# megvii-research/basedet

Hardware: AMD Instinct MI355X
Metric: images/sec training RetinaNet-R50-FPN 1333x800 (higher is better)
Workload: dtype bf16; 1 GPU; retinanet_r50_800x1344 train step (fwd+bwd+allreduce+SGD), DummyLoader boxes, random-init weights, inputs resident in HBM; per_gpu_batch=16, global_batch=16, parallelism=dp1

## Files before the change

basedet_amd/csrc/gskip.hip:

```cpp
#include "common.h"

namespace {

enum { GS_ANY = 1, GS_TOP = 2, GS_BOT = 4, GS_LEFT = 8, GS_RIGHT = 16, GS_TL = 32, GS_TR = 64, GS_BL = 128, GS_BR = 256 };

struct GsSeg { int patch_start, H, W, pw, off; };

struct GsParams {
    const bf16_raw* g;
    int* mask;
    int C, ppi, ph, pw_px, nseg, patches_per_img, total;
    GsSeg seg[BD_MAX_SEGS];
};

__device__ __forceinline__ int gs_level(const GsParams& p, int rem) {
    int s = 0;
#pragma unroll
    for (int k = 1; k < BD_MAX_SEGS; ++k)
        if (k < p.nseg && rem >= p.seg[k].patch_start) s = k;
    return s;
}

__global__ __launch_bounds__(256) void gskip_scan_kernel(const GsParams p) {
    __shared__ int sbits;
    const int tid = threadIdx.x;
    const int pid = blockIdx.x;
    const int n = pid / p.patches_per_img, rem = pid - n * p.patches_per_img;
    const int s = gs_level(p, rem);
    const int H = p.seg[s].H, W = p.seg[s].W, pwn = p.seg[s].pw;
    const int local = rem - p.seg[s].patch_start, by = local / pwn, bx = local - by * pwn;
    const int y0 = by * p.ph, x0 = bx * p.pw_px;
    const int cpp = p.C >> 3;
    const int items = p.ph * p.pw_px * cpp;
    const long long img = (long long)n * p.ppi + p.seg[s].off;
    if (tid == 0) sbits = 0;
    __syncthreads();
    int bits = 0;
    constexpr int U = 8;
    for (int b = 0; b < items; b += 256 * U) {
        u32x4_t v[U];
        int pix[U];
#pragma unroll
        for (int k = 0; k < U; ++k) {
            const int i = b + k * 256 + tid;
            v[k] = (u32x4_t){0u, 0u, 0u, 0u};
            pix[k] = -1;
            if (i < items) {
                const int px = i / cpp, ch = i - px * cpp;
                const int py = px / p.pw_px, pxx = px - py * p.pw_px;
                const int y = y0 + py, x = x0 + pxx;
                if (y < H && x < W) {
                    v[k] = *reinterpret_cast<const u32x4_t*>(p.g + (img + (long long)y * W + x) * p.C + ch * 8);
                    pix[k] = px;
                }
            }
        }
#pragma unroll
        for (int k = 0; k < U; ++k) {
            if (pix[k] >= 0 && (v[k][0] | v[k][1] | v[k][2] | v[k][3])) {
                const int py = pix[k] / p.pw_px, pxx = pix[k] - py * p.pw_px;
                const bool t = py == 0, bo = py == p.ph - 1, l = pxx == 0, r = pxx == p.pw_px - 1;
                bits |= GS_ANY | (t ? GS_TOP : 0) | (bo ? GS_BOT : 0) | (l ? GS_LEFT : 0) | (r ? GS_RIGHT : 0) | (t && l ? GS_TL : 0) |
                        (t && r ? GS_TR : 0) | (bo && l ? GS_BL : 0) | (bo && r ? GS_BR : 0);
            }
        }
    }
#pragma unroll
    for (int m = 32; m >= 1; m >>= 1) bits |= __shfl_xor(bits, m, 64);
    if ((tid & 63) == 0 && bits) atomicOr(&sbits, bits);
    __syncthreads();
    if (tid == 0) p.mask[pid] = sbits;
}

template <bool FRESH>
__device__ __forceinline__ int gs_mask(const int* m, int i) {
    if (FRESH) return __hip_atomic_load(m + i, __ATOMIC_RELAXED, __HIP_MEMORY_SCOPE_AGENT);
    return m[i];
}

template <bool FRESH>
__device__ __forceinline__ void gs_compact_body(const GsParams& p, int* live, int* list, int* count, int* wsum) {
    constexpr int KP = 8;
    const int tid = threadIdx.x, wv = tid >> 6, ln = tid & 63;
    int base = 0;
    for (int c0 = 0; c0 < p.total; c0 += 1024 * KP) {
        int lv[KP];
#pragma unroll
        for (int j = 0; j < KP; ++j) {
            const int q = c0 + tid * KP + j;
            lv[j] = 0;
            if (q < p.total) {
                const int n = q / p.patches_per_img, rem = q - n * p.patches_per_img;
                const int s = gs_level(p, rem);
                const int pwn = p.seg[s].pw, rows = (p.seg[s].H + p.ph - 1) / p.ph;
                const int local = rem - p.seg[s].patch_start, by = local / pwn, bx = local - by * pwn;
                const int* m = p.mask + (long long)n * p.patches_per_img + p.seg[s].patch_start;
                const bool up = by > 0, dn = by + 1 < rows, lf = bx > 0, rt = bx + 1 < pwn;
                int v = gs_mask<FRESH>(m, by * pwn + bx) & GS_ANY;
                if (up) v |= gs_mask<FRESH>(m, (by - 1) * pwn + bx) & GS_BOT;
                if (dn) v |= gs_mask<FRESH>(m, (by + 1) * pwn + bx) & GS_TOP;
                if (lf) v |= gs_mask<FRESH>(m, by * pwn + bx - 1) & GS_RIGHT;
                if (rt) v |= gs_mask<FRESH>(m, by * pwn + bx + 1) & GS_LEFT;
                if (up && lf) v |= gs_mask<FRESH>(m, (by - 1) * pwn + bx - 1) & GS_BR;
                if (up && rt) v |= gs_mask<FRESH>(m, (by - 1) * pwn + bx + 1) & GS_BL;
                if (dn && lf) v |= gs_mask<FRESH>(m, (by + 1) * pwn + bx - 1) & GS_TR;
                if (dn && rt) v |= gs_mask<FRESH>(m, (by + 1) * pwn + bx + 1) & GS_TL;
                lv[j] = v != 0;
            }
        }
        int cnt = 0;
#pragma unroll
        for (int j = 0; j < KP; ++j) cnt += lv[j];
        int inc = cnt;
#pragma unroll
        for (int o = 1; o < 64; o <<= 1) {
            const int y = __shfl_up(inc, o, 64);
            if (ln >= o) inc += y;
        }
        if (ln == 63) wsum[wv] = inc;
        __syncthreads();
        int off = base + inc - cnt, tot = 0;
#pragma unroll
        for (int w = 0; w < 16; ++w) {
            off += w < wv ? wsum[w] : 0;
            tot += wsum[w];
        }
#pragma unroll
        for (int j = 0; j < KP; ++j) {
            const int q = c0 + tid * KP + j;
            if (q < p.total) live[q] = lv[j];
            if (lv[j]) list[off++] = q;
        }
        base += tot;
        __syncthreads();
    }
    if (tid == 0) *count = base;
}

__global__ __launch_bounds__(1024) void gskip_compact_kernel(const GsParams p, int* live, int* list, int* count) {
    __shared__ int wsum[16];
    gs_compact_body<false>(p, live, list, count, wsum);
}

enum { GM_HDR = 8 };

struct GmSeg { int H, W, off, s4, s8, ss; };

struct GmParams {
    const bf16_raw* t;
    const int* live_in;
    int* map;
    int C, ppi, nseg, pi4, pi8, pis, tot4, tot8;
    GmSeg seg[BD_MAX_SEGS];
};

__global__ __launch_bounds__(1024) void gskip_fill_kernel(const GmParams p, const GsParams cp, int total) {
    __shared__ int sbits, slast;
    __shared__ int wsum[16];
    const int tid = threadIdx.x;
    int* m4 = p.map + GM_HDR;
    int* m8 = m4 + p.tot4;
    const int cpp = p.C >> 3;
    const int items = 4 * 16 * cpp;
    for (int pid = blockIdx.x; pid < total; pid += gridDim.x) {
        const int n = pid / p.pis, rem = pid - n * p.pis;
        int s = 0;
#pragma unroll
        for (int k = 1; k < BD_MAX_SEGS; ++k)
            if (k < p.nseg && rem >= p.seg[k].ss) s = k;
        const int H = p.seg[s].H, W = p.seg[s].W;
        const int sc = (W + 15) >> 4, r4 = (H + 3) >> 2, c8 = (W + 7) >> 3;
        const int local = rem - p.seg[s].ss, sy = local / sc, sx = local - sy * sc;
        int q4[2], q8[2];
        bool ok4[2], ok8[2], lv[2];
#pragma unroll
        for (int h = 0; h < 2; ++h) {
            ok4[h] = 2 * sy + h < r4;
            q4[h] = n * p.pi4 + p.seg[s].s4 + (2 * sy + h) * sc + sx;
            ok8[h] = 2 * sx + h < c8;
            q8[h] = n * p.pi8 + p.seg[s].s8 + sy * c8 + 2 * sx + h;
            lv[h] = ok4[h] && (p.live_in == nullptr || p.live_in[q4[h]] != 0);
        }
        int b = 0;
        if (lv[0] || lv[1]) {
            if (tid == 0) sbits = 0;
            __syncthreads();
            const long long img = (long long)n * p.ppi + p.seg[s].off;
            int bits = 0;
#pragma unroll
            for (int h = 0; h < 2; ++h) {
                if (!lv[h]) continue;
                for (int i = tid; i < items; i += 1024) {
                    const int px = i / cpp, ch = i - px * cpp;
                    const int py = px >> 4, pxx = px & 15;
                    const int y = 8 * sy + 4 * h + py, x = 16 * sx + pxx;
                    if (y < H && x < W) {
                        const u32x4_t v = *reinterpret_cast<const u32x4_t*>(p.t + (img + (long long)y * W + x) * p.C + ch * 8);
                        if (v[0] | v[1] | v[2] | v[3]) {
                            const bool t = py == 0, bo = py == 3, l = pxx == 0, r = pxx == 15;
                            const int w = GS_ANY | (t ? GS_TOP : 0) | (bo ? GS_BOT : 0) | (l ? GS_LEFT : 0) | (r ? GS_RIGHT : 0) |
                                          (t && l ? GS_TL : 0) | (t && r ? GS_TR : 0) | (bo && l ? GS_BL : 0) | (bo && r ? GS_BR : 0);
                            bits |= (w << (9 * h)) | (1 << (18 + (pxx >> 3)));
                        }
                    }
                }
            }
#pragma unroll
            for (int m = 32; m >= 1; m >>= 1) bits |= __shfl_xor(bits, m, 64);
            if ((tid & 63) == 0 && bits) atomicOr(&sbits, bits);
            __syncthreads();
            b = sbits;
            __syncthreads();
        }
        if (tid == 0) {
            if (ok4[0]) m4[q4[0]] = b & 511;
            if (ok4[1]) m4[q4[1]] = (b >> 9) & 511;
            if (ok8[0]) m8[q8[0]] = (b >> 18) & 1;
            if (ok8[1]) m8[q8[1]] = (b >> 19) & 1;
        }
    }
    if (tid == 0) {
        __builtin_amdgcn_fence(__ATOMIC_RELEASE, "agent");
        slast = atomicAdd(p.map + 1, 1) == (int)gridDim.x - 1;
    }
    __syncthreads();
    if (!slast) return;
    __builtin_amdgcn_fence(__ATOMIC_ACQUIRE, "agent");
    const int nxt = (p.map[0] & 1) ^ 1;
    int* live = m8 + p.tot8;
    gs_compact_body<true>(cp, live, live + p.tot4 * (1 + nxt), p.map + 2 + nxt, wsum);
    if (tid == 0) { p.map[0] = nxt; p.map[1] = 0; }
}

GsParams gs_params(const bd_conv_desc* d, int ph, int pw, int side = 0) {
    GsParams p{};
    p.C = side ? d->Cin : d->Cout; p.ppi = side ? d->in_pix_per_img : d->out_pix_per_img; p.ph = ph; p.pw_px = pw; p.nseg = d->nseg;
    int ps = 0;
    for (int s = 0; s < d->nseg; ++s) {
        GsSeg& sg = p.seg[s];
        const int H = side ? d->Hi[s] : d->Ho[s], W = side ? d->Wi[s] : d->Wo[s];
        sg.patch_start = ps; sg.H = H; sg.W = W; sg.pw = cdiv(W, pw); sg.off = side ? d->in_off[s] : d->out_off[s];
        ps += cdiv(H, ph) * sg.pw;
    }
    p.patches_per_img = ps;
    p.total = ps * d->N;
    return p;
}

}

int bd_gskip_patches(const bd_conv_desc* d, int ph, int pw) {
    return gs_params(d, ph, pw).total;
}

void bd_gskip_scan(const bd_conv_desc* d, const void* g, int ph, int pw, int* mask, hipStream_t stream) {
    GsParams p = gs_params(d, ph, pw);
    p.g = (const bf16_raw*)g; p.mask = mask;
    if (p.total > 0) hipLaunchKernelGGL(gskip_scan_kernel, dim3(p.total), dim3(256), 0, stream, p);
}

void bd_gskip_compact(const bd_conv_desc* d, int ph, int pw, const int* mask, int* live, int* list, int* count, hipStream_t stream) {
    GsParams p = gs_params(d, ph, pw);
    p.mask = const_cast<int*>(mask);
    hipLaunchKernelGGL(gskip_compact_kernel, dim3(1), dim3(1024), 0, stream, p, live, list, count);
}

void bd_gskip_map_layout(const bd_conv_desc* d, int side, BdGskipMap* out) {
    const int p4 = gs_params(d, 4, 16, side).total, p8 = gs_params(d, 8, 8, side).total;
    out->p4 = p4; out->p8 = p8;
    out->m4 = GM_HDR; out->m8 = GM_HDR + p4; out->live = out->m8 + p8; out->list = out->live + p4;
    out->ints = (size_t)GM_HDR + (size_t)4 * p4 + p8;
}

extern "C" size_t bd_conv2d_gskip_map_bytes(const bd_conv_desc* d, int of_dx) {
    if (!d || d->nseg < 1 || d->nseg > BD_MAX_SEGS || !(d->R == 3 && d->S == 3 && d->stride == 1 && d->pad == 1)) return 0;
    BdGskipMap m;
    bd_gskip_map_layout(d, of_dx ? 1 : 0, &m);
    return m.ints * sizeof(int);
}

void bd_gskip_fill(const bd_conv_desc* d, int side, const void* t, const int* live_in, int* map, hipStream_t stream) {
    const GsParams g4 = gs_params(d, 4, 16, side), g8 = gs_params(d, 8, 8, side), gs = gs_params(d, 8, 16, side);
    GmParams p{};
    p.t = (const bf16_raw*)t; p.live_in = live_in; p.map = map;
    p.C = g4.C; p.ppi = g4.ppi; p.nseg = g4.nseg;
    p.pi4 = g4.patches_per_img; p.pi8 = g8.patches_per_img; p.pis = gs.patches_per_img; p.tot4 = g4.total; p.tot8 = g8.total;
    for (int s = 0; s < g4.nseg; ++s)
        p.seg[s] = GmSeg{g4.seg[s].H, g4.seg[s].W, g4.seg[s].off, g4.seg[s].patch_start, g8.seg[s].patch_start, gs.seg[s].patch_start};
    GsParams cp = g4;
    cp.mask = map + GM_HDR;
    const int grid = gs.total < 128 ? gs.total : 128;
    if (grid > 0) hipLaunchKernelGGL(gskip_fill_kernel, dim3(grid), dim3(1024), 0, stream, p, cp, gs.total);
}

extern "C" int bd_gskip_map_scan(const bd_conv_desc* d, int of_dx, const void* t, void* map, size_t map_bytes, bd_stream_t stream) {
    BD_REQUIRE(d && t && map, "gskip_map_scan: null pointer");
    const size_t need = bd_conv2d_gskip_map_bytes(d, of_dx);
    BD_REQUIRE(need > 0, "gskip_map_scan: liveness maps belong to 3x3 / stride 1 / pad 1 descriptors");
    BD_REQUIRE(map_bytes >= need, "gskip_map_scan: map %zu < required %zu bytes", map_bytes, need);
    const int side = of_dx ? 1 : 0;
    BdGskipMap m;
    bd_gskip_map_layout(d, side, &m);
    int* mp = (int*)map;
    if (hipMemsetAsync(mp, 0, GM_HDR * sizeof(int), (hipStream_t)stream) != hipSuccess) { bd_set_error("gskip_map_scan: memset failed"); return BD_ELAUNCH; }
    GsParams p4 = gs_params(d, 4, 16, side), p8 = gs_params(d, 8, 8, side);
    p4.g = p8.g = (const bf16_raw*)t;
    p4.mask = mp + m.m4; p8.mask = mp + m.m8;
    if (p4.total > 0) {
        hipLaunchKernelGGL(gskip_scan_kernel, dim3(p4.total), dim3(256), 0, (hipStream_t)stream, p4);
        hipLaunchKernelGGL(gskip_scan_kernel, dim3(p8.total), dim3(256), 0, (hipStream_t)stream, p8);
    }
    hipLaunchKernelGGL(gskip_compact_kernel, dim3(1), dim3(1024), 0, (hipStream_t)stream, p4, mp + m.live, mp + m.list, mp + 2);
    BD_CHECK_LAUNCH("bd_gskip_map_scan");
    return BD_OK;
}
```

basedet_amd/layers/modules.py:

```python
import torch

from .. import ops


def _to_nchw(t, N, H, W, C=None):
    v = t.float().view(N, H, W, -1).permute(0, 3, 1, 2).contiguous()
    return v if C is None else v[:, :C].contiguous()


def _level(t, geom, i, C=None):
    N = geom.N
    v = t.view(N, geom.pix_per_img, -1)[:, geom.off[i]: geom.off[i] + geom.H[i] * geom.W[i]]
    return _to_nchw(v.contiguous(), N, geom.H[i], geom.W[i], C)


class _Trunk:
    def __init__(self, cfg, params=None, model=None):
        if model is None:
            from ..models import FCOS, FasterRCNN, RetinaNet
            kind = {"FCOS": FCOS, "ATSS": FCOS, "OTA": FCOS, "FasterRCNN": FasterRCNN}.get(cfg.MODEL.NAME, RetinaNet)
            model = kind(cfg, params=params)
        self.model = model
        self.cfg = cfg

    def _run_trunk(self, image):
        m = self.model
        pre = m.pre_process({"data": image})
        pl = pre["plan"]
        head_forward, m.head_forward = m.head_forward, (lambda _pl: None)
        try:
            m.network_forward(pl)
        finally:
            m.head_forward = head_forward
        return pl


class FPN(_Trunk):

    def __call__(self, image):
        pl = self._run_trunk(image)
        names = self.cfg.MODEL.FPN.OUT_FEATURES
        return {n: _level(pl.P, pl.pyr, i) for i, n in enumerate(names)}

    def output_shape(self):
        ch = self.cfg.MODEL.FPN.OUT_CHANNELS
        return {n: dict(channels=ch, stride=s) for n, s in zip(self.cfg.MODEL.FPN.OUT_FEATURES, self.cfg.MODEL.FPN.STRIDES)}


def build_backbone(cfg, params=None):
    return FPN(cfg, params=params)


class _ResNet(_Trunk):

    def __call__(self, image):
        pl = self._run_trunk(image)
        m = self.model
        out = {}
        for i, blk in enumerate(m.blocks):
            last = i + 1 == len(m.blocks) or m.blocks[i + 1]["layer"] != blk["layer"]
            if last:
                b = pl.blk[i]
                out[f"res{blk['layer'] + 1}"] = _to_nchw(b.out, pl.N, b.gout.H[0], b.gout.W[0])
        return out

    extract_features = __call__


def _resnet(name):
    def make(cfg=None, params=None, **kw):
        from ..configs import RetinaNetConfig
        cfg = cfg or RetinaNetConfig()
        cfg.MODEL.BACKBONE.NAME = name
        if name in ("resnet18", "resnet34"):
            cfg.MODEL.BACKBONE.OUT_FEATURE_CHANNELS = [128, 256, 512]
            cfg.MODEL.FPN.TOP_BLOCK_IN_CHANNELS = 512
        return _ResNet(cfg, params=params)
    make.__name__ = name
    make.__doc__ = f"models/cls/resnet.py: {name} feature extractor (FrozenBN, stem + res2..res5)."
    return make


resnet18, resnet34, resnet50, resnet101 = (_resnet(n) for n in ("resnet18", "resnet34", "resnet50", "resnet101"))


class _Head(_Trunk):
    def _load(self, features):
        m = self.model
        N, _, h0, w0 = features[0].shape
        s0 = m.strides[0]
        pl = m._plan(N, h0 * s0, w0 * s0)
        m._bind_plan(pl)
        assert len(features) == pl.pyr.nlev, "input features expected {}, got {}".format(pl.pyr.nlev, len(features))
        P = pl.P.view(N, pl.pyr.pix_per_img, -1)
        for i, f in enumerate(features):
            assert tuple(f.shape[2:]) == (pl.pyr.H[i], pl.pyr.W[i]), "feature sizes must follow one padded image size"
            P[:, pl.pyr.off[i]: pl.pyr.off[i] + f.shape[2] * f.shape[3]] = \
                f.permute(0, 2, 3, 1).reshape(N, -1, f.shape[1]).to(torch.bfloat16)
        return pl


def _store(dst, geom, grads, C):
    N = geom.N
    v = dst.view(N, geom.pix_per_img, -1)
    v.zero_()
    for i, g in enumerate(grads):
        assert tuple(g.shape[2:]) == (geom.H[i], geom.W[i]) and g.shape[1] == C, "gradient shapes must match the forward outputs"
        v[:, geom.off[i]: geom.off[i] + g.shape[2] * g.shape[3], :C] = g.permute(0, 2, 3, 1).reshape(N, -1, C).to(dst.dtype)


def _real_classes(conv, t):
    if conv.cls_ld == conv.K:
        return t
    return conv.real_logits(t.permute(0, 2, 3, 1)).permute(0, 3, 1, 2).contiguous()


def _pad_classes(conv, g):
    if conv.cls_ld == conv.K:
        return g
    N, _, H, W = g.shape
    out = g.new_zeros((N, conv.A, conv.cls_ld, H, W))
    out[:, :, : conv.K] = g.reshape(N, conv.A, conv.K, H, W)
    return out.reshape(N, conv.A * conv.cls_ld, H, W)


class _HeadBackward:
    def _finish(self, pl):
        m = self.model
        m._join_wgrads()
        torch.cuda.current_stream().synchronize()
        return [_level(pl.g_P, pl.pyr, i) for i in range(pl.pyr.nlev)]

    def grads(self):
        return {k: v for k, v in self.model.reference_grads().items() if k.startswith("head.")}


class RetinaNetHead(_Head, _HeadBackward):

    def __init__(self, cfg, input_shape=None, params=None, model=None):
        super().__init__(cfg, params=params, model=model)

    def __call__(self, features):
        pl = self._load(features)
        m = self.model
        m.head_forward(pl)
        n = pl.pyr.nlev
        self._pl = pl
        return ([_real_classes(m.cls_score, _level(pl.logits, pl.pyr, i)) for i in range(n)],
                [_level(pl.offsets, pl.pyr, i, m.num_anchors * 4) for i in range(n)])

    def backward(self, d_logits, d_offsets):
        pl, m = self._pl, self.model
        m._cur = pl
        m._begin_wgrads()
        assert all(g.shape[1] == m.num_anchors * m.num_classes for g in d_logits), "gradient shapes must match the forward outputs"
        _store(pl.d_logits, pl.pyr, [_pad_classes(m.cls_score, g) for g in d_logits], m.num_anchors * m.cls_ld)
        _store(pl.d_offsets, pl.pyr, d_offsets, m.num_anchors * 4)
        m.head_backward(pl, pl.wgrad_ws, pl.colsum_ws)
        return self._finish(pl)


class PointHead(_Head, _HeadBackward):

    def __init__(self, cfg, input_shape=None, params=None, model=None):
        if model is None:
            from ..models import FCOS
            model = FCOS(cfg, params=params)
        super().__init__(cfg, model=model)

    def __call__(self, features):
        pl = self._load(features)
        self.model.head_forward(pl)
        n = pl.pyr.nlev
        logits = [_level(pl.logits, pl.pyr, i, self.model.num_classes) for i in range(n)]
        offsets = [_level(pl.offsets, pl.pyr, i, 4) for i in range(n)]
        ctr = [_level(pl.raw, pl.pyr, i)[:, 4:5].contiguous() for i in range(n)]
        self._pl = pl
        return logits, offsets, ctr

    def backward(self, d_logits, d_offsets, d_ctrness):
        pl, m = self._pl, self.model
        m._cur = pl
        m._begin_wgrads()
        _store(pl.d_logits, pl.pyr, d_logits, m.num_classes)
        _store(pl.d_off, pl.pyr, d_offsets, 4)
        N = pl.pyr.N
        dc = pl.d_ctr.view(N, pl.pyr.pix_per_img)
        for i, g in enumerate(d_ctrness):
            dc[:, pl.pyr.off[i]: pl.pyr.off[i] + g.shape[2] * g.shape[3]] = g.reshape(N, -1).to(dc.dtype)
        m.head_backward(pl, pl.wgrad_ws, pl.colsum_ws)
        return self._finish(pl)
```

basedet_amd/models/retinanet.py:

```python
import torch

from .. import ops
from ..streams import fork, join
from ..utils.registry import registers
from . import params as P
from .engine import PaddedClsConv
from .fpn_base import FPNDetector, _round_up


@registers.models.register()
class RetinaNet(FPNDetector):
    @staticmethod
    def init_params(cfg, seed=0):
        return P.init_retinanet_params(cfg, seed)

    @classmethod
    def check_config(cls, cfg):
        super().check_config(cfg)
        if not cfg.MODEL.HEAD.get("WITH_NORM", True):
            raise ValueError("MODEL.HEAD.WITH_NORM = False is not supported for the RetinaNet family: only True (the default) is implemented")

    def _build_head(self, add, params):
        m = self.cfg.MODEL
        ch = self.fpn_ch
        self.num_anchors = len(m.ANCHOR.SCALES[0]) * len(m.ANCHOR.RATIOS[0])
        nc = m.HEAD.NUM_CONVS
        self.cls_tower = [add(f"head.cls_subnet.{2 * i}", ch, ch, 3, 1, 1, bias=True) for i in range(nc)]
        self.box_tower = [add(f"head.bbox_subnet.{2 * i}", ch, ch, 3, 1, 1, bias=True) for i in range(nc)]
        A, K = self.num_anchors, self.num_classes
        self.cls_score = self.convs["head.cls_score"] = PaddedClsConv("head.cls_score", ch, A, K, 3, 1, 1, self.device)
        self.cls_ld = self.cls_score.cls_ld
        self.box_ld = _round_up(A * 4, 8)
        self.bbox_pred = add("head.bbox_pred", ch, A * 4, 3, 1, 1, bias=True, cout_pad=self.box_ld)
        if bool(m.get("SPARSE_BOX_BWD", True)) and m.get("WEIGHT_DTYPE", "bf16") == "bf16":
            for c in self.box_tower + [self.bbox_pred]:
                c.gskip = True
        self.sparse_chain = bool(m.get("SPARSE_BOX_CHAIN", True))
        self._build_base_anchors()

    def _head_convs(self):
        return self.cls_tower + self.box_tower + [self.cls_score, self.bbox_pred]

    def _plan_head(self, pl):
        ch = self.fpn_ch
        N = pl.N
        C = pl._carve
        bf = torch.bfloat16

        def act(g, c):
            return C.empty((g.pixels, c), bf)

        nc = len(self.cls_tower)
        pl.cls_act = [act(pl.pyr, ch) for _ in range(nc)]
        pl.box_act = [act(pl.pyr, ch) for _ in range(nc)]
        A, K = self.num_anchors, self.num_classes
        pl.logits = act(pl.pyr, A * self.cls_ld)
        pl.offsets = act(pl.pyr, self.box_ld)
        pl.d_logits = C.like(pl.logits)
        pl.d_offsets = C.like(pl.offsets)
        pl.g_tower = [[act(pl.pyr, ch) for _ in range(nc)] for _ in range(2)]
        pl.g_map = None
        if self.sparse_chain and all(c.gskip for c in self.box_tower + [self.bbox_pred]):
            nb = ops.conv2d_gskip_map_bytes(self.box_tower[0].desc(pl.pyr, pl.pyr))
            if nb:
                pl.g_map = [C.empty(((nb + 3) // 4,), torch.int32) for _ in range(nc)]
        pl.chain_epoch = None
        tw = lambda: C.empty((pl.pyr.pixels, ch), torch.uint8)
        pl.cls_act8 = [tw() if c.fp8 else None for c in self.cls_tower]
        pl.box_act8 = [tw() if c.fp8 else None for c in self.box_tower]
        tg = self.fp8_grad_twins
        pl.g_tower8 = [[tw() if (c.fp8_dgrad and tg) else None for c in tower] for tower in (self.cls_tower, self.box_tower)]
        pl.g_P8 = tw() if (tg and all(t[0].fp8_dgrad for t in (self.cls_tower, self.box_tower))) else None
        self._plan_anchors(pl)
        tot = pl.A_total
        pl.labels = C.empty((N, tot), torch.int32)
        pl.match_idx = C.empty((N, tot), torch.int32)
        pl.gt_offsets = C.empty((N, tot, 4), torch.float32)
        pl.num_fg = C.zeros((1,), torch.int32)
        pl.loss_buf = C.zeros((2,), torch.float32)

    def head_forward(self, pl):
        concurrent = bool(self.cfg.MODEL.get("HEAD_TOWERS_CONCURRENT", True)) and self.weight_dtype != "fp8_e4m3"
        side = self.streams.aux() if concurrent else None
        with fork(side):
            t, t8 = pl.P, getattr(pl, "P8", None)
            for c, a, a8 in zip(self.box_tower, pl.box_act, pl.box_act8):
                c.forward(t, pl.pyr, pl.pyr, a, relu=True, x8=t8, y8=a8); t, t8 = a, a8
            self.bbox_pred.forward(t, pl.pyr, pl.pyr, pl.offsets, x8=t8)
        t, t8 = pl.P, getattr(pl, "P8", None)
        for c, a, a8 in zip(self.cls_tower, pl.cls_act, pl.cls_act8):
            c.forward(t, pl.pyr, pl.pyr, a, relu=True, x8=t8, y8=a8); t, t8 = a, a8
        self.cls_score.forward(t, pl.pyr, pl.pyr, pl.logits, x8=t8)
        join(side)

    def get_losses(self, inputs):
        assert self.training
        pre = self.pre_process(inputs)
        pl = pre["plan"]
        self._cur = pl
        m = self.cfg.MODEL
        gt = pre["gt_boxes"]
        num_gt = pre["img_info"][:, 4].to(torch.int32).contiguous()
        N, Gmax = gt.shape[0], gt.shape[1]
        ws = self._scratch("assign", N * Gmax * 4).view(torch.float32)
        thr = m.MATCHER.THRESHOLDS
        side = self.streams.aux() if m.get("ASSIGN_ON_SIDE_STREAM", True) else None
        with fork(side):
            ops.retina_assign_encode(pl.anchors, gt, num_gt, thr[0], thr[1], m.MATCHER.ALLOW_LOW_QUALITY, m.BOX_REG.MEAN,
                                     m.BOX_REG.STD, pl.labels, pl.match_idx, pl.gt_offsets, pl.num_fg, ws)
        self.network_forward(pl)
        join(side)
        pl.loss_buf.zero_()
        rows = N * pl.A_total
        ops.focal_loss_fwd_bwd(pl.logits, pl.labels, rows, self.num_classes, m.LOSSES.FOCAL_LOSS_ALPHA,
                               m.LOSSES.FOCAL_LOSS_GAMMA, pl.num_fg, 1.0, pl.loss_buf[0:1], pl.d_logits,
                               ld=self.cls_ld if self.cls_ld != self.num_classes else None)
        ops.smooth_l1_fwd_bwd(pl.offsets, pl.gt_offsets, pl.labels, pl.pyr.pixels, self.num_anchors, self.box_ld,
                              m.LOSSES.SMOOTH_L1_BETA, pl.num_fg, m.LOSSES.REG_LOSS_WEIGHT, pl.loss_buf[1:2], pl.d_offsets)
        cls_loss, reg_loss = pl.loss_buf[0], pl.loss_buf[1]
        return {"total_loss": cls_loss + reg_loss, "cls_loss": cls_loss, "reg_loss": reg_loss}

    def head_backward(self, pl, ws, cws):
        pyr = pl.pyr
        for ti, (tower, acts, pred, dpred) in enumerate(((self.cls_tower, pl.cls_act, self.cls_score, pl.d_logits),
                                                         (self.box_tower, pl.box_act, self.bbox_pred, pl.d_offsets))):
            gbuf, g8 = pl.g_tower[ti], pl.g_tower8[ti]
            n = len(tower)
            maps = pl.g_map if (ti == 1 and self.sparse_chain and all(c.gskip for c in tower + [pred])) else None
            if ti == 1:
                clean = maps is not None and pl.chain_epoch == self.plan_arena.epoch
                pl.chain_epoch = self.plan_arena.epoch if maps is not None else None
                if maps is not None:
                    pred.set_chain(None, maps[n - 1], clean)
                    for i in range(n):
                        tower[i].set_chain(maps[i], maps[i - 1] if i > 0 else None, clean)
            gs = tower[n - 1].grad_scale
            self._wgrad(pred, acts[-1], dpred, pyr, pyr, ws, cws)
            tw = g8[n - 1] if pred.dgrad_writes_twin(pyr, pyr) else None
            if not pred.dgrad(dpred, pyr, pyr, gbuf[n - 1], mask=acts[-1], dx8=tw, q_scale=gs):
                tw = None
            act8 = pl.cls_act8 if ti == 0 else pl.box_act8
            for i in range(n - 1, -1, -1):
                x = acts[i - 1] if i > 0 else pl.P
                x8 = (act8[i - 1] if i > 0 else pl.P8) if tw is not None else None
                self._wgrad(tower[i], x, gbuf[i], pyr, pyr, ws, cws, x8=x8, g8=tw)
                if i > 0:
                    nxt = g8[i - 1] if tower[i].dgrad_writes_twin(pyr, pyr) else None
                    wrote = tower[i].dgrad(gbuf[i], pyr, pyr, gbuf[i - 1], mask=acts[i - 1], g8=tw, dx8=nxt, q_scale=tower[i - 1].grad_scale)
                    tw = nxt if wrote else None
                else:
                    wrote_p = tower[i].dgrad(gbuf[i], pyr, pyr, pl.g_P, first=(ti == 0), g8=tw,
                                             dx8=pl.g_P8 if tower[i].dgrad_writes_twin(pyr, pyr) else None,
                                             q_scale=self.output[self.fpn_stages[0]].grad_scale)
        for c in self.box_tower + [self.bbox_pred]:
            c.set_chain()
        pl.g_P8_ready = pl.g_P8 is not None and bool(wrote_p)

    def _debug_head(self, pl, out, lvl):
        for i in range(pl.pyr.nlev):
            for k in range(len(self.cls_tower)):
                out[f"cls{k}_{i}"] = lvl(pl.cls_act[k], i)
                out[f"box{k}_{i}"] = lvl(pl.box_act[k], i)
            lg = lvl(pl.logits, i)
            out[f"logits_{i}"] = self.cls_score.real_logits(lg.permute(0, 2, 3, 1)).permute(0, 3, 1, 2).contiguous()
            out[f"offs_{i}"] = lvl(pl.offsets, i, self.num_anchors * 4)

    def inference_batch(self, inputs):
        assert not self.training
        pre = self.pre_process(inputs)
        pl = pre["plan"]
        self.network_forward(pl)
        K, A = self.num_classes, self.num_anchors
        m = self.cfg.MODEL
        return self._detect(pl.N, [h * w * A for h, w in pl.sizes], K, 0, pre["img_info"], logits=pl.logits, anchors=pl.anchors,
                            offsets=pl.offsets, off_ld=self.box_ld, A=A, mean=m.BOX_REG.MEAN, std=m.BOX_REG.STD, cls_ld=self.cls_ld)
```

Before: 685.5 images/sec.

## Scan box-regression gradient liveness once after loss and feed it to bbox_pred chain

Rewrites the gskip fill kernel so each wave handles its own range of patches, reads activations with unrolled vector loads, and writes dead patches directly instead of using block-wide syncs per patch. The standalone map scan now calls this single fused fill kernel in place of two scan kernels plus a compaction kernel. The retinanet head scans the sparse d_offsets gradient right after the loss and passes that map to bbox_pred's chain, which previously got no input map, so its dgrad can skip zero-gradient tiles. The cost is an extra scan kernel in the forward/loss phase plus extra map memory.

```diff
diff --git a/basedet_amd/csrc/gskip.hip b/basedet_amd/csrc/gskip.hip
--- a/basedet_amd/csrc/gskip.hip
+++ b/basedet_amd/csrc/gskip.hip
@@ -142,7 +142,7 @@
     gs_compact_body<false>(p, live, list, count, wsum);
 }
 
-enum { GM_HDR = 8 };
+enum { GM_HDR = 8, GM_WAVES = 16, GM_MAX_GRID = 128, GM_U = 8 };
 
 struct GmSeg { int H, W, off, s4, s8, ss; };
 
@@ -151,19 +151,27 @@
     const int* live_in;
     int* map;
     int C, ppi, nseg, pi4, pi8, pis, tot4, tot8;
+    int per_wave;
     GmSeg seg[BD_MAX_SEGS];
 };
 
-__global__ __launch_bounds__(1024) void gskip_fill_kernel(const GmParams p, const GsParams cp, int total) {
-    __shared__ int sbits, slast;
+__global__ __launch_bounds__(64 * GM_WAVES) void gskip_fill_kernel(const GmParams p, const GsParams cp, int total) {
+    __shared__ int slast;
     __shared__ int wsum[16];
-    const int tid = threadIdx.x;
+    const int tid = threadIdx.x, lane = tid & 63;
     int* m4 = p.map + GM_HDR;
     int* m8 = m4 + p.tot4;
     const int cpp = p.C >> 3;
-    const int items = 4 * 16 * cpp;
-    for (int pid = blockIdx.x; pid < total; pid += gridDim.x) {
-        const int n = pid / p.pis, rem = pid - n * p.pis;
+    const int step_px = 64 / cpp, step_ch = 64 - step_px * cpp;
+    const int px_l = lane / cpp, ch_l = lane - px_l * cpp;
+    const int wave = blockIdx.x * GM_WAVES + (tid >> 6);
+    const long long b0 = (long long)wave * p.per_wave;
+    const int b1 = (int)(b0 + p.per_wave < total ? b0 + p.per_wave : total);
+    for (int c0 = (int)(b0 < total ? b0 : total); c0 < b1; c0 += 64) {
+        const int pid = c0 + lane;
+        const bool valid = pid < b1;
+        const int pd = valid ? pid : c0;
+        const int n = pd / p.pis, rem = pd - n * p.pis;
         int s = 0;
 #pragma unroll
         for (int k = 1; k < BD_MAX_SEGS; ++k)
@@ -171,54 +179,72 @@
         const int H = p.seg[s].H, W = p.seg[s].W;
         const int sc = (W + 15) >> 4, r4 = (H + 3) >> 2, c8 = (W + 7) >> 3;
         const int local = rem - p.seg[s].ss, sy = local / sc, sx = local - sy * sc;
-        int q4[2], q8[2];
-        bool ok4[2], ok8[2], lv[2];
-#pragma unroll
-        for (int h = 0; h < 2; ++h) {
-            ok4[h] = 2 * sy + h < r4;
-            q4[h] = n * p.pi4 + p.seg[s].s4 + (2 * sy + h) * sc + sx;
-            ok8[h] = 2 * sx + h < c8;
-            q8[h] = n * p.pi8 + p.seg[s].s8 + sy * c8 + 2 * sx + h;
-            lv[h] = ok4[h] && (p.live_in == nullptr || p.live_in[q4[h]] != 0);
-        }
-        int b = 0;
-        if (lv[0] || lv[1]) {
-            if (tid == 0) sbits = 0;
-            __syncthreads();
-            const long long img = (long long)n * p.ppi + p.seg[s].off;
+        const int q4 = n * p.pi4 + p.seg[s].s4 + 2 * sy * sc + sx;
+        const int q8 = n * p.pi8 + p.seg[s].s8 + sy * c8 + 2 * sx;
+        const bool ok4b = 2 * sy + 1 < r4, ok8b = 2 * sx + 1 < c8;
+        int lv = 0;
+        if (valid) {
+            if (p.live_in == nullptr) lv = ok4b ? 3 : 1;
+            else {
+                const int f0 = p.live_in[q4], f1 = ok4b ? p.live_in[q4 + sc] : 0;
+                lv = (f0 != 0 ? 1 : 0) | (f1 != 0 ? 2 : 0);
+            }
+            if (lv == 0) {
+                m4[q4] = 0;
+                if (ok4b) m4[q4 + sc] = 0;
+                m8[q8] = 0;
+                if (ok8b) m8[q8 + 1] = 0;
+            }
+        }
+        unsigned long long todo = __ballot(lv != 0);
+        while (todo) {
+            const int j = __builtin_amdgcn_readfirstlane(__ffsll((long long)todo) - 1);
+            todo &= todo - 1;
+            const int jn = __builtin_amdgcn_readfirstlane(__shfl(n, j, 64)), js = __builtin_amdgcn_readfirstlane(__shfl(s, j, 64));
+            const int jsy = __builtin_amdgcn_readfirstlane(__shfl(sy, j, 64)), jsx = __builtin_amdgcn_readfirstlane(__shfl(sx, j, 64));
+            const int jlv = __builtin_amdgcn_readfirstlane(__shfl(lv, j, 64));
+            const int jH = p.seg[js].H, jW = p.seg[js].W;
+            const int y0 = 8 * jsy, x0 = 16 * jsx;
+            const bf16_raw* base = p.t + ((long long)jn * p.ppi + p.seg[js].off) * p.C;
+            const int kbeg = (jlv & 1) ? 0 : cpp, kend = (jlv & 2) ? 2 * cpp : cpp;
+            int px = px_l + (kbeg ? 64 : 0), ch = ch_l;
             int bits = 0;
-#pragma unroll
-            for (int h = 0; h < 2; ++h) {
-                if (!lv[h]) continue;
-                for (int i = tid; i < items; i += 1024) {
-                    const int px = i / cpp, ch = i - px * cpp;
-                    const int py = px >> 4, pxx = px & 15;
-                    const int y = 8 * sy + 4 * h + py, x = 16 * sx + pxx;
-                    if (y < H && x < W) {
-                        const u32x4_t v = *reinterpret_cast<const u32x4_t*>(p.t + (img + (long long)y * W + x) * p.C + ch * 8);
-                        if (v[0] | v[1] | v[2] | v[3]) {
-                            const bool t = py == 0, bo = py == 3, l = pxx == 0, r = pxx == 15;
-                            const int w = GS_ANY | (t ? GS_TOP : 0) | (bo ? GS_BOT : 0) | (l ? GS_LEFT : 0) | (r ? GS_RIGHT : 0) |
-                                          (t && l ? GS_TL : 0) | (t && r ? GS_TR : 0) | (bo && l ? GS_BL : 0) | (bo && r ? GS_BR : 0);
-                            bits |= (w << (9 * h)) | (1 << (18 + (pxx >> 3)));
-                        }
+            for (int k0 = kbeg; k0 < kend; k0 += GM_U) {
+                u32x4_t v[GM_U];
+                int vpx[GM_U];
+#pragma unroll
+                for (int u = 0; u < GM_U; ++u) {
+                    v[u] = (u32x4_t){0u, 0u, 0u, 0u};
+                    vpx[u] = px;
+                    const int y = y0 + (px >> 4), x = x0 + (px & 15);
+                    if (k0 + u < kend && y < jH && x < jW)
+                        v[u] = *reinterpret_cast<const u32x4_t*>(base + ((long long)y * jW + x) * p.C + ch * 8);
+                    px += step_px; ch += step_ch;
+                    if (ch >= cpp) { ch -= cpp; ++px; }
+                }
+#pragma unroll
+                for (int u = 0; u < GM_U; ++u) {
+                    if (v[u][0] | v[u][1] | v[u][2] | v[u][3]) {
+                        const int h = vpx[u] >> 6, py = (vpx[u] >> 4) & 3, pxx = vpx[u] & 15;
+                        const bool t = py == 0, bo = py == 3, l = pxx == 0, r = pxx == 15;
+                        const int w = GS_ANY | (t ? GS_TOP : 0) | (bo ? GS_BOT : 0) | (l ? GS_LEFT : 0) | (r ? GS_RIGHT : 0) |
+                                      (t && l ? GS_TL : 0) | (t && r ? GS_TR : 0) | (bo && l ? GS_BL : 0) | (bo && r ? GS_BR : 0);
+                        bits |= (w << (9 * h)) | (1 << (18 + (pxx >> 3)));
                     }
                 }
             }
 #pragma unroll
             for (int m = 32; m >= 1; m >>= 1) bits |= __shfl_xor(bits, m, 64);
-            if ((tid & 63) == 0 && bits) atomicOr(&sbits, bits);
-            __syncthreads();
-            b = sbits;
-            __syncthreads();
-        }
-        if (tid == 0) {
-            if (ok4[0]) m4[q4[0]] = b & 511;
-            if (ok4[1]) m4[q4[1]] = (b >> 9) & 511;
-            if (ok8[0]) m8[q8[0]] = (b >> 18) & 1;
-            if (ok8[1]) m8[q8[1]] = (b >> 19) & 1;
-        }
-    }
+            if (lane == j) {
+                m4[q4] = bits & 511;
+                if (ok4b) m4[q4 + sc] = (bits >> 9) & 511;
+                m8[q8] = (bits >> 18) & 1;
+                if (ok8b) m8[q8 + 1] = (bits >> 19) & 1;
+            }
+        }
+    }
+    asm volatile("s_waitcnt vmcnt(0)" ::: "memory");
+    __syncthreads();
     if (tid == 0) {
         __builtin_amdgcn_fence(__ATOMIC_RELEASE, "agent");
         slast = atomicAdd(p.map + 1, 1) == (int)gridDim.x - 1;
@@ -289,8 +315,12 @@
         p.seg[s] = GmSeg{g4.seg[s].H, g4.seg[s].W, g4.seg[s].off, g4.seg[s].patch_start, g8.seg[s].patch_start, gs.seg[s].patch_start};
     GsParams cp = g4;
     cp.mask = map + GM_HDR;
-    const int grid = gs.total < 128 ? gs.total : 128;
-    if (grid > 0) hipLaunchKernelGGL(gskip_fill_kernel, dim3(grid), dim3(1024), 0, stream, p, cp, gs.total);
+    int grid = cdiv(gs.total, 2 * GM_WAVES);
+    if (grid > GM_MAX_GRID) grid = GM_MAX_GRID;
+    if (grid > 0) {
+        p.per_wave = cdiv(gs.total, grid * GM_WAVES);
+        hipLaunchKernelGGL(gskip_fill_kernel, dim3(grid), dim3(64 * GM_WAVES), 0, stream, p, cp, gs.total);
+    }
 }
 
 extern "C" int bd_gskip_map_scan(const bd_conv_desc* d, int of_dx, const void* t, void* map, size_t map_bytes, bd_stream_t stream) {
@@ -298,19 +328,10 @@
     const size_t need = bd_conv2d_gskip_map_bytes(d, of_dx);
     BD_REQUIRE(need > 0, "gskip_map_scan: liveness maps belong to 3x3 / stride 1 / pad 1 descriptors");
     BD_REQUIRE(map_bytes >= need, "gskip_map_scan: map %zu < required %zu bytes", map_bytes, need);
-    const int side = of_dx ? 1 : 0;
-    BdGskipMap m;
-    bd_gskip_map_layout(d, side, &m);
+    BD_REQUIRE((of_dx ? d->Cin : d->Cout) % 8 == 0, "gskip_map_scan: %d channels are no multiple of 8", of_dx ? d->Cin : d->Cout);
     int* mp = (int*)map;
-    if (hipMemsetAsync(mp, 0, GM_HDR * sizeof(int), (hipStream_t)stream) != hipSuccess) { bd_set_error("gskip_map_scan: memset failed"); return BD_ELAUNCH; }
-    GsParams p4 = gs_params(d, 4, 16, side), p8 = gs_params(d, 8, 8, side);
-    p4.g = p8.g = (const bf16_raw*)t;
-    p4.mask = mp + m.m4; p8.mask = mp + m.m8;
-    if (p4.total > 0) {
-        hipLaunchKernelGGL(gskip_scan_kernel, dim3(p4.total), dim3(256), 0, (hipStream_t)stream, p4);
-        hipLaunchKernelGGL(gskip_scan_kernel, dim3(p8.total), dim3(256), 0, (hipStream_t)stream, p8);
-    }
-    hipLaunchKernelGGL(gskip_compact_kernel, dim3(1), dim3(1024), 0, (hipStream_t)stream, p4, mp + m.live, mp + m.list, mp + 2);
+    if (hipMemsetAsync(mp + 1, 0, sizeof(int), (hipStream_t)stream) != hipSuccess) { bd_set_error("gskip_map_scan: memset failed"); return BD_ELAUNCH; }
+    bd_gskip_fill(d, of_dx ? 1 : 0, t, nullptr, mp, (hipStream_t)stream);
     BD_CHECK_LAUNCH("bd_gskip_map_scan");
     return BD_OK;
 }
diff --git a/basedet_amd/layers/modules.py b/basedet_amd/layers/modules.py
--- a/basedet_amd/layers/modules.py
+++ b/basedet_amd/layers/modules.py
@@ -156,6 +156,7 @@
         assert all(g.shape[1] == m.num_anchors * m.num_classes for g in d_logits), "gradient shapes must match the forward outputs"
         _store(pl.d_logits, pl.pyr, [_pad_classes(m.cls_score, g) for g in d_logits], m.num_anchors * m.cls_ld)
         _store(pl.d_offsets, pl.pyr, d_offsets, m.num_anchors * 4)
+        pl.d_map_fresh = False
         m.head_backward(pl, pl.wgrad_ws, pl.colsum_ws)
         return self._finish(pl)
 
diff --git a/basedet_amd/models/retinanet.py b/basedet_amd/models/retinanet.py
--- a/basedet_amd/models/retinanet.py
+++ b/basedet_amd/models/retinanet.py
@@ -36,6 +36,7 @@
             for c in self.box_tower + [self.bbox_pred]:
                 c.gskip = True
         self.sparse_chain = bool(m.get("SPARSE_BOX_CHAIN", True))
+        self.dmap_late = bool(m.get("SPARSE_BOX_DMAP_LATE", False))
         self._build_base_anchors()
 
     def _head_convs(self):
@@ -59,11 +60,13 @@
         pl.d_logits = C.like(pl.logits)
         pl.d_offsets = C.like(pl.offsets)
         pl.g_tower = [[act(pl.pyr, ch) for _ in range(nc)] for _ in range(2)]
-        pl.g_map = None
+        pl.g_map = pl.d_map = None
         if self.sparse_chain and all(c.gskip for c in self.box_tower + [self.bbox_pred]):
             nb = ops.conv2d_gskip_map_bytes(self.box_tower[0].desc(pl.pyr, pl.pyr))
-            if nb:
+            nd = ops.conv2d_gskip_map_bytes(self.bbox_pred.desc(pl.pyr, pl.pyr))
+            if nb and nd:
                 pl.g_map = [C.empty(((nb + 3) // 4,), torch.int32) for _ in range(nc)]
+                pl.d_map = C.empty(((nd + 3) // 4,), torch.int32)
         pl.chain_epoch = None
         tw = lambda: C.empty((pl.pyr.pixels, ch), torch.uint8)
         pl.cls_act8 = [tw() if c.fp8 else None for c in self.cls_tower]
@@ -117,8 +120,16 @@
                                ld=self.cls_ld if self.cls_ld != self.num_classes else None)
         ops.smooth_l1_fwd_bwd(pl.offsets, pl.gt_offsets, pl.labels, pl.pyr.pixels, self.num_anchors, self.box_ld,
                               m.LOSSES.SMOOTH_L1_BETA, pl.num_fg, m.LOSSES.REG_LOSS_WEIGHT, pl.loss_buf[1:2], pl.d_offsets)
+        pl.d_map_fresh = False
+        if not self.dmap_late:
+            self._scan_d_offsets(pl)
         cls_loss, reg_loss = pl.loss_buf[0], pl.loss_buf[1]
         return {"total_loss": cls_loss + reg_loss, "cls_loss": cls_loss, "reg_loss": reg_loss}
+
+    def _scan_d_offsets(self, pl):
+        if pl.d_map is not None:
+            ops.gskip_map_scan(self.bbox_pred.desc(pl.pyr, pl.pyr), pl.d_offsets, pl.d_map)
+            pl.d_map_fresh = True
 
     def head_backward(self, pl, ws, cws):
         pyr = pl.pyr
@@ -131,7 +142,10 @@
                 clean = maps is not None and pl.chain_epoch == self.plan_arena.epoch
                 pl.chain_epoch = self.plan_arena.epoch if maps is not None else None
                 if maps is not None:
-                    pred.set_chain(None, maps[n - 1], clean)
+                    if not getattr(pl, "d_map_fresh", False):
+                        self._scan_d_offsets(pl)
+                    pl.d_map_fresh = False
+                    pred.set_chain(pl.d_map, maps[n - 1], clean)
                     for i in range(n):
                         tower[i].set_chain(maps[i], maps[i - 1] if i > 0 else None, clean)
             gs = tower[n - 1].grad_scale
```

Result: no change. 687.4 images/sec, median of 6 (+0.3%).
